# jianwang-mpi/SceneEgo

Measured on NVIDIA B200. Metric: frames/s VoxelNetDepth volumetric stage, higher is better.
Workload: dtype bf16

## Files before the change

sceneego_b200/build.py:

```python
import concurrent.futures
import hashlib
import os
import subprocess
import sys

HERE = os.path.dirname(os.path.abspath(__file__))
CSRC = os.path.join(HERE, "csrc")
LIB = os.path.join(HERE, "libsceneego_b200.so")
LIB_F16 = os.path.join(HERE, "libsceneego_b200_f16.so")
HASH_FILE = LIB + ".srchash"
OBJ_DIR = os.path.join(HERE, "build")
SOURCES = ["geometry.cu", "softargmax.cu", "v2v.cu", "stem.cu", "stem_march.cu", "tail.cu", "march.cu", "eval.cu", "handoff.cu", "feature_conv.cu"]
NVCC_FLAGS = ["-gencode", "arch=compute_100a,code=sm_100a", "-O3", "-lineinfo", "-std=c++17",
              "-Xcompiler", "-fPIC", "-Xptxas", "-v"]


def _sources():
    return [s for s in SOURCES if os.path.exists(os.path.join(CSRC, s))]


def source_hash() -> str:
    h = hashlib.sha256()
    deps = sorted(os.path.join(CSRC, f) for f in os.listdir(CSRC) if f.endswith((".cu", ".cuh", ".h")))
    deps.append(os.path.join(HERE, "..", "include", "sceneego_b200.h"))
    for d in deps:
        h.update(os.path.basename(d).encode())
        h.update(open(d, "rb").read())
    h.update(" ".join(NVCC_FLAGS + _sources()).encode())
    return h.hexdigest()


def recorded_hash() -> str:
    try:
        return open(HASH_FILE).read().strip()
    except OSError:
        return ""


def _stale() -> bool:
    return not (os.path.exists(LIB) and os.path.exists(LIB_F16)) or recorded_hash() != source_hash()


VARIANTS = [("bf16", LIB, []), ("f16", LIB_F16, ["-DSCENEEGO_ACT_F16"])]


# ... 40 lines not shown
```

sceneego_b200/csrc/common.cuh:

```cuda
#pragma once
#include <cuda_runtime.h>
#include <cuda_bf16.h>
#include <cuda_fp16.h>
#include <stdint.h>
#include <stdio.h>
#include "../../include/sceneego_b200.h"

namespace sceneego {

#ifdef SCENEEGO_ACT_F16
constexpr int kActDtype = 1;
constexpr uint32_t kIdescAB = 0u;
#define SE_MMA_SYNC_AB ".f16.f16"
__device__ __forceinline__ uint32_t act_pack2(float lo, float hi) {
  uint32_t r;
  asm("cvt.rn.satfinite.f16x2.f32 %0, %1, %2;" : "=r"(r) : "f"(hi), "f"(lo));
  return r;
}
__device__ __forceinline__ uint32_t act_pack2_relu(float lo, float hi) {
  uint32_t r;
  asm("cvt.rn.relu.satfinite.f16x2.f32 %0, %1, %2;" : "=r"(r) : "f"(hi), "f"(lo));
  return r;
}
__device__ __forceinline__ float2 act_unpack2(uint32_t u) { return __half22float2(*reinterpret_cast<const __half2*>(&u)); }
// ... 62 lines not shown
}

__device__ __forceinline__ float voxel_coord(float lo, float step, int i) {
  return __fadd_rn(lo, __fmul_rn(step, (float)i));
}

__host__ __device__ inline int64_t vol_cell(const sceneego_vol_layout_t& L, int b, int x, int y, int z, int g, int C8) {
  if (L.s2d) {
    const int par = ((x & 1) << 2) | ((y & 1) << 1) | (z & 1);
    return (int64_t)(par * C8 + g) * L.plane_stride + vol_pos(L, b, x >> 1, y >> 1, z >> 1);
  }
  return (int64_t)g * L.plane_stride + vol_pos(L, b, x, y, z);
}
__host__ __device__ inline int64_t vol_scene_elem(const sceneego_vol_layout_t& L, int b, int x, int y, int z, int C8) {
  if (L.s2d) {
    const int par = ((x & 1) << 2) | ((y & 1) << 1) | (z & 1);
    return ((int64_t)(8 * C8) * L.plane_stride + vol_pos(L, b, x >> 1, y >> 1, z >> 1)) * 8 + par;
  }
  return ((int64_t)C8 * L.plane_stride + vol_pos(L, b, x, y, z)) * 8;
}

constexpr int kNumSMs = 148;

int launch_stem_s2d(const sceneego_v2v_op_t& op, void* const* d_buffers, const void* d_blob, int batch, int op_index,
                    bool simt, cudaStream_t st);
int launch_feature_conv1x1_simt(const float* d_feat, const float* d_weight, const float* d_bias, float* d_out, int batch,
                                int cin, int cout, int h, int w, cudaStream_t st);
int launch_stem_march(const sceneego_v2v_op_t& op, void* const* d_buffers, const void* d_blob, int batch, int op_index,
                      bool simt, cudaStream_t st);
int launch_tail_mlp(const sceneego_v2v_op_t& op, void* const* d_buffers, const void* d_blob, int batch, int op_index,
                    bool simt, cudaStream_t st);
int launch_conv_march(const sceneego_v2v_op_t& op, void* const* d_buffers, const void* d_blob, int batch, int op_index,
                      cudaStream_t st);

}
```

sceneego_b200/csrc/v2v.cu:

```cuda
#include "tc_common.cuh"
#include <stdarg.h>
#include <stdlib.h>
#include <string.h>
#include <math.h>
#include <mutex>

namespace sceneego {


struct ConvParams {
  const __nv_bfloat16* src;
  __nv_bfloat16* dst;
  const __nv_bfloat16* res;
  float* dst_f32;
  const __nv_bfloat16* w;
  const float* bias;
  sceneego_vol_layout_t ls, ld;
  int batch;
  int k, r, cin_planes, ksteps, N, cout_real, flags;
  int xs, n0, n_dx, n_xg, items_per_plane;
  FastDiv fd_frame, fd_px, fd_py;
  int deconv, par0;
  int taps_dx;
  int mma_n;
  int tiles, L, WL;
  int n_items;
  int win_stages, w_slots, wchunk_taps, wchunks_per_dx;
  int wrows;
  uint32_t win_bytes, wchunk_bytes, tap_bytes;
  uint32_t off_win, off_w, off_bias, off_bar;
  uint32_t tmem_cols, half_cols;
  int cg;
  uint32_t w_half_bytes;
  const __nv_bfloat16* src2;
  int n_dx2;
  uint32_t w_main_bytes;
  int march;
  int n0_shift;
};

constexpr int CONV_EPI_WARPS = 8;
__host__ __device__ constexpr int conv_mma_warps(int tiles) { return tiles >= 4 ? 4 : tiles; }
__host__ __device__ constexpr int conv_threads(int tiles) { return 32 * (1 + conv_mma_warps(tiles) + CONV_EPI_WARPS); }
constexpr int CONV_MAX_THREADS = 32 * (1 + 4 + CONV_EPI_WARPS);
constexpr int MAX_STAGES = 4, MAX_WSLOTS = 8;

struct RowInfo {
  bool write;
  bool valid;
  int b, n;
  int x, y, z;
  int64_t dpos;
};

__device__ __forceinline__ RowInfo decode_row(const ConvParams& p, int64_t q64) {
  RowInfo ri;
  ri.write = false; ri.valid = false; ri.b = 0; ri.n = 0; ri.dpos = 0; ri.x = ri.y = ri.z = 0;
  const int S = p.ls.side;
  const uint32_t q = (uint32_t)q64;
  const uint32_t b = fdiv(q, p.fd_frame);
  const int rem = (int)(q - b * (uint32_t)p.ls.frame_pitch) - p.ls.guard;
  if ((int)b >= p.batch || rem < 0) return ri;
  const int x = (int)fdiv((uint32_t)rem, p.fd_px);
  const int r2 = rem - x * p.ls.pitch_x;
  const int y = (int)fdiv((uint32_t)r2, p.fd_py);
  const int z = r2 - y * p.ls.pitch_y;
  if (x >= S) return ri;
  if (y >= S + p.ld.pad || z >= S + p.ld.pad) return ri;
  ri.write = true;
  ri.valid = (y < S) && (z < S);
  ri.b = (int)b;
  ri.x = x; ri.y = y; ri.z = z;
  ri.n = (x * S + y) * S + z;
  const int m = p.deconv ? 2 : 1;
  ri.dpos = (int64_t)b * p.ld.frame_pitch + p.ld.guard + (int64_t)(m * x) * p.ld.pitch_x + (int64_t)(m * y) * p.ld.pitch_y + m * z;
  return ri;
}

__device__ __forceinline__ RowInfo decode_row_plane(const ConvParams& p, int b, int x, int cell) {
  RowInfo ri;
  ri.write = false; ri.valid = false; ri.b = b; ri.n = 0; ri.dpos = 0; ri.x = x; ri.y = ri.z = 0;
  const int S = p.ls.side;
  if (cell >= p.ls.pitch_x) return ri;
  const int y = (int)fdiv((uint32_t)cell, p.fd_py);
  const int z = cell - y * p.ls.pitch_y;
  if (y >= S + p.ld.pad || z >= S + p.ld.pad) return ri;
  ri.write = true;
  ri.valid = (y < S) && (z < S);
  ri.y = y; ri.z = z;
  ri.n = (x * S + y) * S + z;
  ri.dpos = (int64_t)b * p.ld.frame_pitch + p.ld.guard + (int64_t)x * p.ld.pitch_x + (int64_t)y * p.ld.pitch_y + z;
  return ri;
}

__device__ __forceinline__ void store_row16_pre(const ConvParams& p, const RowInfo& ri, int c0, float (&v)[16],
                                                const float* s_bias, const uint4& r0, const uint4& r1) {
  if (!ri.write) return;
  const int S = p.ls.side;
  if (p.flags & SCENEEGO_F_OUT_F32) {
    if (!ri.valid) return;
    const size_t N3 = (size_t)S * S * S;
#pragma unroll
    for (int j = 0; j < 16; ++j) {
      const int c = c0 + j;
      if (c < p.cout_real) {
        float o = v[j] + s_bias[c];
        if (p.flags & SCENEEGO_F_RELU) o = fmaxf(o, 0.f);
        p.dst_f32[((size_t)ri.b * p.cout_real + c) * N3 + ri.n] = o;
// ... 172 lines not shown
          }
          for (int e = 0; e < p.n_dx2; ++e) {
            mbar_wait(BAR(B_FULL_WIN + ws), wph);
            mbar_arrive_remote(mapa_shared(BAR(B_FULL_WIN + ws), 0));
            if (++ws == p.win_stages) { ws = 0; wph ^= 1; }
            mbar_wait(BAR(B_FULL_W + sl), sph);
            mbar_arrive_remote(mapa_shared(BAR(B_FULL_W + sl), 0));
            if (++sl == p.w_slots) { sl = 0; sph ^= 1; }
          }
        }
      }
    } else {
    const uint32_t tmem_u = __shfl_sync(0xffffffffu, tmem_base, 0);
    const bool leader = elect_one();
    auto WAIT = [&](uint32_t bar, uint32_t parity) {
      if constexpr (CG == 2) mbar_wait_warp_cluster(bar, parity); else mbar_wait_warp(bar, parity);
    };
    auto MMA = [&](uint32_t d, uint64_t a, uint64_t b, uint32_t id, uint32_t ac) {
      if constexpr (CG == 2) tc_mma_bf16_pair(d, a, b, id, ac); else tc_mma_bf16(d, a, b, id, ac);
    };
    auto COMMIT = [&](uint32_t bar) {
      if constexpr (CG == 2) tc_commit_pair(bar); else tc_commit(bar);
    };
    const uint32_t idesc = (1u << 4) | kIdescAB | ((uint32_t)(p.mma_n >> 3) << 17) | ((CG == 2 ? 16u : 8u) << 24);
    const uint64_t desc_hi = (uint64_t)(8u | (1u << 14)) << 32;
    const uint32_t a_lo_flags = ((p.win_bytes >> 4) & 0x3FFFu) << 16;
    const uint32_t n_mine = (uint32_t)p.mma_n / CG;
    const uint32_t b_lo_flags = ((n_mine * 16u >> 4) & 0x3FFFu) << 16;
    const uint32_t a_ks_step = (2u * p.win_bytes) >> 4;
    const uint32_t b_ks_step = (2u * n_mine * 16u) >> 4;
    const uint32_t b_tap_step = p.tap_bytes >> 4;
    const uint32_t n_cols = (uint32_t)p.N;
    const int pitch_y = p.ls.pitch_y, ksz = p.k, wtaps = p.wchunk_taps;
    const uint32_t is_deconv = (uint32_t)p.deconv, par_cols = (uint32_t)p.n0;
    const uint32_t my_tile = (uint32_t)(warp - 1);
    const uint32_t a_mine = my_tile * 128u;
    int ws = 0, wph = 0, sl = 0, sph = 0;
    for (int it = 0; it < my_items; ++it) {
      const int buf = it & 1;
      WAIT(BAR(B_TMEM_EMPTY + buf), ((it >> 1) & 1) ^ 1);
      tc_fence_after();
      const uint32_t d_mine = tmem_u + (uint32_t)buf * p.half_cols + my_tile * n_cols;
      uint32_t acc = 0;
      for (int dx = 0; dx < p.n_dx; ++dx) {
        WAIT(BAR(B_FULL_WIN + ws), wph);
        const uint32_t win_lo = (((sbase + p.off_win + (uint32_t)(ws * 2 * KSTEPS) * p.win_bytes) >> 4) & 0x3FFFu) |
                                a_lo_flags;
        int dy = 0, dz = 0;
        uint32_t dcol = 0;
        for (int wc = 0; wc < p.wchunks_per_dx; ++wc) {
          WAIT(BAR(B_FULL_W + sl), sph);
          tc_fence_after();
          uint32_t b_lo = (((sbase + p.off_w + (uint32_t)sl * p.wchunk_bytes) >> 4) & 0x3FFFu) | b_lo_flags;
          if constexpr (WROWS == 0) {
            for (int tp = 0; tp < wtaps; ++tp) {
              const uint32_t a_lo = win_lo + (uint32_t)(dy * pitch_y + dz);
              if (leader) {
#pragma unroll
                for (int tt = 0; tt < TILES / NW; ++tt) {
#pragma unroll
                  for (int ks = 0; ks < KSTEPS; ++ks)
                    MMA(d_mine + (uint32_t)(tt * NW) * n_cols + dcol,
                                desc_hi | (a_lo + a_mine + (uint32_t)(tt * NW) * 128u + (uint32_t)ks * a_ks_step),
                                desc_hi | (b_lo + (uint32_t)ks * b_ks_step), idesc, ks == 0 ? acc : 1u);
                }
              }
              b_lo += b_tap_step;
              if (is_deconv) { dcol += par_cols; }
              else { acc = 1; if (++dz == ksz) { dz = 0; ++dy; } }
            }
          } else {
            if (leader) {
#pragma unroll
              for (int r = 0; r < WROWS; ++r) {
                const uint32_t a_row = win_lo + a_mine + (uint32_t)((dy + r) * pitch_y);
#pragma unroll
                for (int j = 0; j < 3; ++j) {
#pragma unroll
                  for (int tt = 0; tt < TILES / NW; ++tt) {
#pragma unroll
                    for (int ks = 0; ks < KSTEPS; ++ks)
                      MMA(d_mine + (uint32_t)(tt * NW) * n_cols,
                                  desc_hi | (a_row + (uint32_t)j + (uint32_t)(tt * NW) * 128u + (uint32_t)ks * a_ks_step),
                                  desc_hi | (b_lo + (uint32_t)(r * 3 + j) * b_tap_step + (uint32_t)ks * b_ks_step), idesc,
                                  (ks == 0 && r == 0 && j == 0) ? acc : 1u);
                  }
                }
              }
            }
            acc = 1;
            dy += WROWS;
          }
          if (leader) COMMIT(BAR(B_EMPTY_W + sl));
          if (++sl == p.w_slots) { sl = 0; sph ^= 1; }
        }
        if (leader) COMMIT(BAR(B_EMPTY_WIN + ws));
        if (++ws == p.win_stages) { ws = 0; wph ^= 1; }
      }
      if constexpr (KSTEPS % 2 == 0) {
        for (int e = 0; e < p.n_dx2; ++e) {
          WAIT(BAR(B_FULL_WIN + ws), wph);
          WAIT(BAR(B_FULL_W + sl), sph);
          tc_fence_after();
          const uint32_t a_c = ((((sbase + p.off_win + (uint32_t)(ws * 2 * KSTEPS) * p.win_bytes) >> 4) & 0x3FFFu) | a_lo_flags) +
                               a_mine + (uint32_t)(p.r * (pitch_y + 1));
          const uint32_t b_c = (((sbase + p.off_w + (uint32_t)sl * p.wchunk_bytes) >> 4) & 0x3FFFu) | b_lo_flags;
          if (leader) {
#pragma unroll
            for (int tt = 0; tt < TILES / NW; ++tt) {
#pragma unroll
              for (int ks = 0; ks < KSTEPS / 2; ++ks)
                MMA(d_mine + (uint32_t)(tt * NW) * n_cols, desc_hi | (a_c + (uint32_t)(tt * NW) * 128u + (uint32_t)ks * a_ks_step),
                    desc_hi | (b_c + (uint32_t)ks * b_ks_step), idesc, 1u);
            }
          }
          if (leader) COMMIT(BAR(B_EMPTY_W + sl));
          if (++sl == p.w_slots) { sl = 0; sph ^= 1; }
          if (leader) COMMIT(BAR(B_EMPTY_WIN + ws));
          if (++ws == p.win_stages) { ws = 0; wph ^= 1; }
        }
      }
      if (leader) COMMIT(BAR(B_TMEM_FULL + buf));
    }
    __syncwarp();
    }
  } else {
    const int quarter = warp & 3;
    const int half = (warp - FIRST_EPI) >> 2;
    const int nch = p.N >> 4;
    const int S = p.ls.side;
    const int t_first = TILES >= 2 ? half : 0, t_step = TILES >= 2 ? 2 : 1;
    const int c_first = TILES >= 2 ? 0 : half, c_step = TILES >= 2 ? 1 : 2;
    auto shifted = [&](const RowInfo& ri, int x0, int c, int& ch0) -> RowInfo {
      if (XS == 1 && p.deconv) {
        const int blk = p.n0_shift >= 0 ? ((c << 4) >> p.n0_shift) : (c << 4) / p.n0;
        const int par = p.par0 + blk;
        ch0 = (c << 4) - blk * p.n0;
        RowInfo r = ri;
        r.write = ri.valid;
        r.dpos = ri.dpos + ((par >> 2) * p.ld.pitch_x + ((par >> 1) & 1) * p.ld.pitch_y + (par & 1));
        return r;
      }
      if (XS == 1) { ch0 = c << 4; return ri; }
      const int sft = p.n0_shift >= 0 ? ((c << 4) >> p.n0_shift) : (c << 4) / p.n0;
      ch0 = (c << 4) - sft * p.n0;
      RowInfo r = ri;
      const bool in = (x0 + sft) < S;
      r.write = ri.write && in;
      r.valid = ri.valid && in;
      r.dpos = ri.dpos + (int64_t)sft * p.ld.pitch_x;
      r.n = ri.n + sft * S * S;
      return r;
    };
    for (int it = 0; it < my_items; ++it) {
      const int buf = it & 1;
      int ib, ix0, icell0;
      const int64_t q0 = item_origin(item_of(it), ib, ix0, icell0);
      auto row_info = [&](int t) -> RowInfo {
        const int r = t * 128 + quarter * 32 + lane;
        return XS == 1 ? decode_row(p, q0 + r) : decode_row_plane(p, ib, ix0, icell0 + r);
      };
      RowInfo ri = row_info(t_first);
      if constexpr (TILES == 1) {
        constexpr int D = 4;
        uint4 q0r[D], q1r[D];
#pragma unroll
        for (int d = 0; d < D; ++d) {
          q0r[d] = make_uint4(0, 0, 0, 0); q1r[d] = q0r[d];
          const int c = c_first + d * c_step;
          if (c < nch) { int chn; const RowInfo rp = shifted(ri, ix0, c, chn); load_res16(p, rp, chn, q0r[d], q1r[d]); }
        }
        mbar_wait(BAR(B_TMEM_FULL + buf), (it >> 1) & 1);
        tc_fence_after();
        const uint32_t taddr = tmem_base + ((uint32_t)(quarter * 32) << 16) + (uint32_t)buf * p.half_cols;
        int cpf = c_first + D * c_step;
// ... 165 lines not shown
  const int So = ld.side;
  const int n = blockIdx.x * blockDim.x + threadIdx.x;
  const int g = blockIdx.y, b = blockIdx.z;
  if (n >= So * So * So || g >= planes) return;
  const int z = n % So, y = (n / So) % So, x = n / (So * So);
  float m[8];
#pragma unroll
  for (int j = 0; j < 8; ++j) m[j] = -INFINITY;
#pragma unroll
  for (int t = 0; t < 8; ++t) {
    const int64_t q = vol_pos(ls, b, 2 * x + (t >> 2), 2 * y + ((t >> 1) & 1), 2 * z + (t & 1));
    float a[8];
    unpack8(*reinterpret_cast<const uint4*>(src + ((int64_t)g * ls.plane_stride + q) * 8), a);
#pragma unroll
    for (int j = 0; j < 8; ++j) m[j] = fmaxf(m[j], a[j]);
  }
  *reinterpret_cast<uint4*>(dst + ((int64_t)g * ld.plane_stride + vol_pos(ld, b, x, y, z)) * 8) = pack8(m);
}

__global__ void __launch_bounds__(128) deconv2_kernel(const __grid_constant__ ConvParams p) {
  const int So = p.ld.side;
  const int n = blockIdx.x * blockDim.x + threadIdx.x;
  const int go = blockIdx.y, b = blockIdx.z;
  if (n >= So * So * So) return;
  const int z = n % So, y = (n / So) % So, x = n / (So * So);
  const int tap = ((x & 1) * 2 + (y & 1)) * 2 + (z & 1);
  const int64_t qs = vol_pos(p.ls, b, x >> 1, y >> 1, z >> 1);
  float acc[8];
#pragma unroll
  for (int j = 0; j < 8; ++j) acc[j] = 0.f;
  for (int g = 0; g < p.cin_planes; ++g) {
    float a[8];
    unpack8(*reinterpret_cast<const uint4*>(p.src + ((int64_t)g * p.ls.plane_stride + qs) * 8), a);
    int npar = 256 / p.N;
    if (npar > 8) npar = 8;
    const uint4* wrow = reinterpret_cast<const uint4*>(p.w) +
                        ((size_t)(tap / npar) * p.cin_planes + g) * ((size_t)npar * p.N) + (size_t)(tap % npar) * p.N + go * 8;
#pragma unroll
    for (int j = 0; j < 8; ++j) {
      float wv[8];
      unpack8(__ldg(wrow + j), wv);
#pragma unroll
      for (int i = 0; i < 8; ++i) acc[j] = fmaf(a[i], wv[i], acc[j]);
    }
  }
  const int64_t cell = (int64_t)go * p.ld.plane_stride + vol_pos(p.ld, b, x, y, z);
  float rr[8];
  if (p.flags & SCENEEGO_F_ADD_AFTER) unpack8(*reinterpret_cast<const uint4*>(p.res + cell * 8), rr);
#pragma unroll
  for (int j = 0; j < 8; ++j) {
    float t = acc[j] + p.bias[go * 8 + j];
    if (p.flags & SCENEEGO_F_RELU) t = fmaxf(t, 0.f);
    if (p.flags & SCENEEGO_F_ADD_AFTER) t += rr[j];
    acc[j] = t;
  }
  *reinterpret_cast<uint4*>(p.dst + cell * 8) = pack8(acc);
}

static thread_local char g_err[512] = "";
int ensure_max_dynamic_smem(const void* kernel, int bytes) {
  struct Entry { int dev; const void* fn; int bytes; };
  static Entry seen[512];
  static int n_seen = 0;
  static std::mutex mu;
  int dev = 0;
  cudaError_t e = cudaGetDevice(&dev);
  if (e != cudaSuccess) { set_error("cudaGetDevice: %s", cudaGetErrorString(e)); return SCENEEGO_E_CUDA; }
  std::lock_guard<std::mutex> lock(mu);
  for (int i = 0; i < n_seen; ++i)
    if (seen[i].dev == dev && seen[i].fn == kernel && seen[i].bytes >= bytes) return SCENEEGO_OK;
  e = cudaFuncSetAttribute(kernel, cudaFuncAttributeMaxDynamicSharedMemorySize, bytes);
  if (e != cudaSuccess) { set_error("cudaFuncSetAttribute(MaxDynamicSharedMemorySize): %s", cudaGetErrorString(e)); return SCENEEGO_E_CUDA; }
  if (n_seen < 512) seen[n_seen++] = Entry{dev, kernel, bytes};
  return SCENEEGO_OK;
}

void set_error(const char* fmt, ...) {
  va_list ap;
  va_start(ap, fmt);
  vsnprintf(g_err, sizeof(g_err), fmt, ap);
  va_end(ap);
}
static thread_local int g_launches = 0;

static bool try_plan(ConvParams& p, int tiles, int want_stages) {
  const int taps_dx = p.taps_dx;
  const int L = tiles * 128;
  const int WL = L + 2 * p.r * (p.ls.pitch_y + 1);
  const uint32_t win_bytes = (uint32_t)WL * 16u;
  const uint32_t stage = win_bytes * p.cin_planes;
  const uint32_t fixed = 1024;
  if ((uint64_t)stage * want_stages + fixed > kMaxSmem) return false;
  const uint32_t used = stage * want_stages + fixed;
  const uint32_t room = kMaxSmem - used;
  int wct = taps_dx, wrows = 0;
  if (p.k == 3 && !p.deconv && 3u * 9u * p.tap_bytes <= room) { wct = 9; wrows = 3; }
  else if (p.k == 3 && !p.deconv && 2u * 3u * p.tap_bytes <= room) { wct = 3; wrows = 1; }
  else {
    while (wct > 1 && (uint32_t)wct * p.tap_bytes > 24576u) {
      int nx = wct - 1;
      while (nx > 1 && taps_dx % nx) --nx;
      wct = nx;
    }
  }
  { const char* e = getenv("SCENEEGO_WCHUNK"); if (e && atoi(e) > 0 && taps_dx % atoi(e) == 0) { wct = atoi(e); wrows = (p.k == 3 && !p.deconv && wct % 3 == 0) ? wct / 3 : 0; if (wrows == 2) wrows = 0; } }
  const uint32_t wchunk = (uint32_t)wct * p.tap_bytes;
  if (2ull * wchunk > room) return false;
  int slots = (int)(room / wchunk);
  if (slots > MAX_WSLOTS) slots = MAX_WSLOTS;
  if (slots > 4 && wchunk > 8192) slots = 4;
  { const char* e = getenv("SCENEEGO_WSLOTS"); if (e && atoi(e) >= 2 && atoi(e) <= MAX_WSLOTS && (uint64_t)used + (uint64_t)atoi(e) * wchunk <= kMaxSmem) slots = atoi(e); }
  p.wrows = wrows;
  p.tiles = tiles; p.L = L; p.WL = WL;
  p.win_bytes = win_bytes; p.win_stages = want_stages;
  p.wchunk_taps = wct; p.wchunks_per_dx = taps_dx / wct; p.wchunk_bytes = wchunk; p.w_slots = slots;
  p.off_win = 0;
  p.off_w = stage * want_stages;
  p.off_bias = p.off_w + wchunk * slots;
  p.off_bar = p.off_bias + 512;
  p.half_cols = (uint32_t)(tiles * p.N);
  uint32_t cols = 32;
  while (cols < 2 * p.half_cols) cols <<= 1;
  p.tmem_cols = cols;
  return true;
}

static int plan_conv(ConvParams& p, int64_t n_pos) {
  p.tap_bytes = (uint32_t)p.cin_planes * (p.mma_n / p.cg) * 16u;
  int max_tiles = 256 / p.N;
  if (max_tiles > 8) max_tiles = 8;
  if (p.xs == 1 && p.cg == 1) {
    auto items_of = [&](int t) { return (n_pos + (int64_t)t * 128 - 1) / ((int64_t)t * 128); };
    if (items_of(max_tiles) < 4 * kNumSMs) {
      int best = max_tiles;
      int64_t best_cost = ((items_of(max_tiles) + kNumSMs - 1) / kNumSMs) * max_tiles;
      for (int t = max_tiles >> 1; t >= 1; t >>= 1) {
        const int64_t cost = ((items_of(t) + kNumSMs - 1) / kNumSMs) * t;
        if (cost < best_cost) { best_cost = cost; best = t; }
// ... 26 lines not shown
extern "C" int sceneego_v2v_last_launch_count(void) { return g_launches; }

extern "C" int sceneego_v2v_pack_conv(const float* h_weight, const float* h_bias, const float* h_gamma,
                                      const float* h_beta, const float* h_mean, const float* h_var, double eps,
                                      int cout, int cin, int ksize, int transposed, int cout_pad, int cin_pad,
                                      int xstack, int n_split, uint16_t* h_w_out, float* h_b_out) {
  SE_REQUIRE(h_weight && h_w_out && h_b_out, "pack_conv: null argument");
  SE_REQUIRE(cout_pad >= cout && cin_pad >= cin && cout_pad % 8 == 0 && cin_pad % 8 == 0, "pack_conv: bad padding");
  SE_REQUIRE(xstack >= 1 && (xstack == 1 || !transposed), "pack_conv: bad xstack");
  SE_REQUIRE(n_split == 1 || (n_split == 2 && !transposed && (xstack * cout_pad) % 32 == 0), "pack_conv: bad n_split");
  const int taps = ksize * ksize * ksize;
  const int kk = ksize * ksize;
  const int n_stk = xstack * cout_pad;
  const int n_dx = ksize + xstack - 1;
  memset(h_w_out, 0, (size_t)n_dx * kk * cin_pad * n_stk * sizeof(uint16_t));
  for (int co = 0; co < cout_pad; ++co) {
    double scale = 1.0, shift = 0.0;
    if (co < cout) {
      if (h_gamma) {
        scale = (double)h_gamma[co] / sqrt((double)h_var[co] + eps);
        shift = (double)h_beta[co] - (double)h_mean[co] * scale;
      }
      h_b_out[co] = (float)((h_bias ? (double)h_bias[co] : 0.0) * scale + shift);
    } else {
      h_b_out[co] = 0.f;
    }
    if (co >= cout) continue;
    for (int ci = 0; ci < cin; ++ci)
      for (int t = 0; t < taps; ++t) {
        const size_t src = transposed ? (((size_t)ci * cout + co) * taps + t) : (((size_t)co * cin + ci) * taps + t);
        const uint16_t wv = f2bf((float)((double)h_weight[src] * scale));
        const int dx = t / kk, rest = t % kk;
        if (transposed) {
          int npar = 256 / cout_pad;
          if (npar > 8) npar = 8;
          const size_t grp = (size_t)t / npar, nrow = (size_t)(t % npar) * cout_pad + co;
          h_w_out[((grp * (cin_pad / 8) + ci / 8) * ((size_t)npar * cout_pad) + nrow) * 8 + (ci & 7)] = wv;
          continue;
        }
        for (int sft = 0; sft < xstack; ++sft) {
          const size_t tp = (size_t)(dx + sft) * kk + rest;
          const size_t col = (size_t)sft * cout_pad + co;
          const size_t nh = (size_t)n_stk / n_split, hf = col / nh;
          const size_t half_elems = (size_t)n_dx * kk * cin_pad * nh;
          const size_t dst = hf * half_elems + ((tp * (cin_pad / 8) + ci / 8) * nh + (col - hf * nh)) * 8 + (ci & 7);
          h_w_out[dst] = wv;
        }
      }
  }
  return SCENEEGO_OK;
}

static int launch_conv_tc(ConvParams& p, int batch, int op_index, cudaStream_t st) {
  p.n0_shift = -1;
  for (int k = 3; k < 10; ++k) if ((1 << k) == p.n0) p.n0_shift = k;
  const int64_t n_pos = (int64_t)batch * p.ls.frame_pitch;
  SE_REQUIRE(n_pos + 4096 < (1ll << 31) && (n_pos + 4096) * (int64_t)p.ls.frame_pitch < (1ll << 48),
             "v2v_run: op %d: batch * frame_pitch too large for one launch (use a smaller chunk)", op_index);
  p.fd_frame = make_fastdiv((uint32_t)p.ls.frame_pitch);
  p.fd_px = make_fastdiv((uint32_t)p.ls.pitch_x);
  p.fd_py = make_fastdiv((uint32_t)p.ls.pitch_y);
  const int smem = plan_conv(p, n_pos);
  SE_REQUIRE(smem > 0, "v2v_run: op %d does not fit shared memory", op_index);
  if (p.xs == 1) {
    p.n_items = (int)((n_pos + p.L - 1) / p.L);
  } else {
    p.items_per_plane = (p.ls.pitch_x + p.L - 1) / p.L;
    p.n_xg = (p.ls.side + p.xs - 1) / p.xs;
// ... 45 lines not shown
    ConvParams p;
    memset(&p, 0, sizeof(p));
    p.src = (const __nv_bfloat16*)d_buffers[op.src];
    p.dst = (__nv_bfloat16*)d_buffers[op.dst];
    p.dst_f32 = (float*)d_buffers[op.dst];
    p.res = op.res >= 0 ? (const __nv_bfloat16*)d_buffers[op.res] : nullptr;
    p.ls = op.lay_src; p.ld = op.lay_dst; p.batch = batch; p.flags = op.flags;
    SE_REQUIRE(p.src && p.dst, "v2v_run: op %d has a null buffer", i);
    SE_REQUIRE(!(op.flags & (SCENEEGO_F_RESIDUAL | SCENEEGO_F_ADD_AFTER)) || p.res, "v2v_run: op %d needs a residual", i);
    if (op.type == SCENEEGO_OP_MAXPOOL2) {
      SE_REQUIRE(op.lay_dst.side * 2 == op.lay_src.side && op.cin % 8 == 0, "v2v_run: op %d bad pool shape", i);
      const int So = op.lay_dst.side;
      dim3 grid((So * So * So + 255) / 256, op.cin / 8, batch);
      maxpool2_kernel<<<grid, 256, 0, st>>>(p.src, p.dst, p.ls, p.ld, op.cin / 8);
      SE_CUDA_LAUNCH_CHECK("maxpool2");
      ++g_launches;
      continue;
    }
    if (op.type == SCENEEGO_OP_STEM7_S2D || op.type == SCENEEGO_OP_TAIL_MLP || op.type == SCENEEGO_OP_STEM7_MARCH) {
      const bool simt = op.impl == 1 || force_simt;
      const int rc = op.type == SCENEEGO_OP_STEM7_S2D ? launch_stem_s2d(op, d_buffers, d_blob, batch, i, simt, st)
                     : op.type == SCENEEGO_OP_STEM7_MARCH ? launch_stem_march(op, d_buffers, d_blob, batch, i, simt, st)
                                                          : launch_tail_mlp(op, d_buffers, d_blob, batch, i, simt, st);
      if (rc != SCENEEGO_OK) return rc;
      ++g_launches;
      continue;
    }
    p.w = (const __nv_bfloat16*)((const char*)d_blob + op.w_offset);
    p.bias = (const float*)((const char*)d_blob + op.b_offset);
    p.cin_planes = op.cin / 8; p.ksteps = op.cin / 16; p.N = op.cout; p.cout_real = op.cout_real;
    p.xs = 1; p.n0 = op.cout; p.n_dx = op.ksize; p.n_xg = 0; p.items_per_plane = 0; p.cg = 1;
    if (op.type == SCENEEGO_OP_DECONV2) {
      SE_REQUIRE(op.lay_dst.side == 2 * op.lay_src.side && op.cin % 8 == 0 && op.cout % 8 == 0, "v2v_run: op %d bad deconv shape", i);
      if (op.impl == 1 || force_simt || op.cin % 16 || op.cout % 16 || op.cout > 256) {
        const int So = op.lay_dst.side;
        dim3 grid((So * So * So + 127) / 128, op.cout / 8, batch);
        deconv2_kernel<<<grid, 128, 0, st>>>(p);
        SE_CUDA_LAUNCH_CHECK("deconv2");
        ++g_launches;
        continue;
      }
      int npar = 256 / op.cout;
      if (npar > 8) npar = 8;
      const __nv_bfloat16* w_all = p.w;
      for (int par0 = 0; par0 < 8; par0 += npar) {
        ConvParams q = p;
        q.k = 1; q.r = 0; q.xs = 1; q.n0 = op.cout; q.mma_n = npar * op.cout; q.N = npar * op.cout; q.n_dx = 1;
        q.deconv = 1; q.par0 = par0; q.taps_dx = 1;
        q.w = w_all + (size_t)par0 * q.cin_planes * op.cout * 8;
        const int rc = launch_conv_tc(q, batch, i, st);
        if (rc != SCENEEGO_OK) return rc;
      }
      continue;
    }
    if (op.type == SCENEEGO_OP_CONV3_MARCH) {
      if (op.impl == 1 || force_simt) {
        SE_REQUIRE(op.ksize == 3 && op.cin % 16 == 0 && op.cout % 16 == 0, "v2v_run: op %d bad marching conv", i);
        p.k = 3; p.r = 1; p.xs = 1; p.n0 = op.cout; p.N = op.cout; p.cg = 1; p.march = 1;
        p.fd_frame = make_fastdiv((uint32_t)p.ls.frame_pitch);
        p.fd_px = make_fastdiv((uint32_t)p.ls.pitch_x);
        p.fd_py = make_fastdiv((uint32_t)p.ls.pitch_y);
        p.src2 = nullptr; p.n_dx2 = 0;
        if (op.src2 >= 0 && op.cin2 > 0) { p.src2 = (const __nv_bfloat16*)d_buffers[op.src2]; p.n_dx2 = 1; }
        p.w_main_bytes = 27u * (uint32_t)p.cin_planes * (uint32_t)op.cout * 16u;
        p.w_half_bytes = 0;
        const int64_t n_pos = (int64_t)batch * p.ls.frame_pitch;
        dim3 grid((unsigned)((n_pos + 127) / 128), op.cout / 16);
        conv_simt_kernel<<<grid, 128, 0, st>>>(p, n_pos);
        SE_CUDA_LAUNCH_CHECK("conv_simt (march layout)");
      } else {
        const int rc = launch_conv_march(op, d_buffers, d_blob, batch, i, st);
        if (rc != SCENEEGO_OK) return rc;
      }
      ++g_launches;
      continue;
    }
    SE_REQUIRE(op.type == SCENEEGO_OP_CONV, "v2v_run: op %d unknown type", i);
    SE_REQUIRE(op.ksize == 1 || op.ksize == 3 || op.ksize == 7, "v2v_run: op %d unsupported kernel size", i);
    SE_REQUIRE(op.cin % 16 == 0 && op.cout % 16 == 0 && op.cout >= 16 && op.cout <= 128, "v2v_run: op %d channels must be multiples of 16", i);
    SE_REQUIRE(op.lay_src.side == op.lay_dst.side && op.lay_src.pad >= op.ksize / 2 && op.lay_dst.pad <= op.lay_src.pad,
               "v2v_run: op %d layouts incompatible with the stencil", i);
    p.k = op.ksize; p.r = op.ksize / 2;
    const int64_t n_pos = (int64_t)batch * p.ls.frame_pitch;
    p.fd_frame = make_fastdiv((uint32_t)p.ls.frame_pitch);
    p.fd_px = make_fastdiv((uint32_t)p.ls.pitch_x);
    p.fd_py = make_fastdiv((uint32_t)p.ls.pitch_y);
    p.cg = op.cta_pair == 2 ? 2 : 1;
    p.src2 = nullptr; p.n_dx2 = 0;
    if (op.src2 >= 0 && op.cin2 > 0) {
      SE_REQUIRE(op.cin2 * 2 == op.cin && (op.cin / 16) % 2 == 0 && op.ksize == 3 && d_buffers[op.src2],
                 "v2v_run: op %d: a fused shortcut needs a 3^3 conv and a second source with half its channels", i);
      p.src2 = (const __nv_bfloat16*)d_buffers[op.src2];
      p.n_dx2 = op.xstack > 1 ? op.xstack : 1;
    }
    if (op.impl == 1 || force_simt) {
      const int xs_ = op.xstack > 1 ? op.xstack : 1;
      p.n0 = op.cout; p.N = xs_ * op.cout;
      const uint32_t tapb = (uint32_t)p.cin_planes * (p.N / p.cg) * 16u;
      p.w_main_bytes = (uint32_t)((op.ksize + xs_ - 1) * op.ksize * op.ksize) * tapb;
      p.w_half_bytes = p.w_main_bytes + (uint32_t)p.n_dx2 * (tapb / 2);
      dim3 grid((unsigned)((n_pos + 127) / 128), op.cout / 16);
      conv_simt_kernel<<<grid, 128, 0, st>>>(p, n_pos);
      SE_CUDA_LAUNCH_CHECK("conv_simt");
      ++g_launches;
      continue;
    }
    const int xs = op.xstack > 1 ? op.xstack : 1;
    SE_REQUIRE(xs * op.cout <= 256, "v2v_run: op %d: xstack * cout exceeds 256 columns", i);
    SE_REQUIRE(p.cg == 1 || (xs * op.cout) % 32 == 0, "v2v_run: op %d: a CTA pair splits N in halves of whole 16-column groups", i);
    p.xs = xs; p.n0 = op.cout; p.N = xs * op.cout; p.mma_n = p.N; p.n_dx = op.ksize + xs - 1;
    p.deconv = 0; p.par0 = 0; p.taps_dx = op.ksize * op.ksize;
    const int rc = launch_conv_tc(p, batch, i, st);
    if (rc != SCENEEGO_OK) return rc;
  }
  if (ev) cudaEventRecord(ev[n_ops], st);
  return SCENEEGO_OK;
}

extern "C" int sceneego_v2v_run(const sceneego_v2v_op_t* ops, int n_ops, void* const* d_buffers, const void* d_blob,
                                int batch, void* stream) {
  return v2v_run_impl(ops, n_ops, d_buffers, d_blob, batch, stream, nullptr);
}

extern "C" int sceneego_v2v_run_profile(const sceneego_v2v_op_t* ops, int n_ops, void* const* d_buffers,
                                        const void* d_blob, int batch, void* stream, float* h_ms) {
  SE_REQUIRE(h_ms && n_ops > 0 && n_ops < 4096, "v2v_run_profile: bad argument");
  cudaEvent_t* ev = (cudaEvent_t*)malloc(sizeof(cudaEvent_t) * (n_ops + 1));
  for (int i = 0; i <= n_ops; ++i) cudaEventCreate(&ev[i]);
  int rc = v2v_run_impl(ops, n_ops, d_buffers, d_blob, batch, stream, ev);
  if (rc == SCENEEGO_OK) {
    cudaError_t e = cudaEventSynchronize(ev[n_ops]);
    if (e != cudaSuccess) { set_error("v2v_run_profile: %s", cudaGetErrorString(e)); rc = SCENEEGO_E_CUDA; }
    for (int i = 0; i < n_ops && rc == SCENEEGO_OK; ++i) cudaEventElapsedTime(&h_ms[i], ev[i], ev[i + 1]);
  }
  for (int i = 0; i <= n_ops; ++i) cudaEventDestroy(ev[i]);
  free(ev);
  return rc;
}
```

Measured before the change: 2992.

## Add dedicated warp-specialized tcgen05 transposed-conv kernel with smem-staged bulk stores

Replaces the per-parity-group launches of the generic tensor-core conv for 2x transposed convolutions with one persistent warp-specialized kernel. A producer warp streams input windows, weights and optional residual tiles through mbarrier pipelines, and an MMA warp accumulates into double-buffered TMEM. Sixteen epilogue warps scatter results into a shared-memory output image that a storer warp writes back with bulk async copies. The aim is to cut multiple launches, reread source data less often and coalesce the strided parity writes. The cost is considerable new synchronization complexity and a deconv path removed from the generic kernel.

```diff
diff --git a/sceneego_b200/build.py b/sceneego_b200/build.py
--- a/sceneego_b200/build.py
+++ b/sceneego_b200/build.py
@@ -10,7 +10,7 @@
 LIB_F16 = os.path.join(HERE, "libsceneego_b200_f16.so")
 HASH_FILE = LIB + ".srchash"
 OBJ_DIR = os.path.join(HERE, "build")
-SOURCES = ["geometry.cu", "softargmax.cu", "v2v.cu", "stem.cu", "stem_march.cu", "tail.cu", "march.cu", "eval.cu", "handoff.cu", "feature_conv.cu"]
+SOURCES = ["geometry.cu", "softargmax.cu", "v2v.cu", "stem.cu", "stem_march.cu", "tail.cu", "march.cu", "eval.cu", "handoff.cu", "feature_conv.cu", "deconv.cu"]
 NVCC_FLAGS = ["-gencode", "arch=compute_100a,code=sm_100a", "-O3", "-lineinfo", "-std=c++17",
               "-Xcompiler", "-fPIC", "-Xptxas", "-v"]
 
diff --git a/sceneego_b200/csrc/common.cuh b/sceneego_b200/csrc/common.cuh
--- a/sceneego_b200/csrc/common.cuh
+++ b/sceneego_b200/csrc/common.cuh
@@ -118,5 +118,8 @@
                     bool simt, cudaStream_t st);
 int launch_conv_march(const sceneego_v2v_op_t& op, void* const* d_buffers, const void* d_blob, int batch, int op_index,
                       cudaStream_t st);
+__host__ __device__ inline int deconv_npar(int cout) { return 256 / cout < 8 ? 256 / cout : 8; }
+int launch_deconv_tc(const sceneego_v2v_op_t& op, void* const* d_buffers, const void* d_blob, int batch, int op_index,
+                     cudaStream_t st);
 
 }
diff --git a/sceneego_b200/csrc/deconv.cu b/sceneego_b200/csrc/deconv.cu
--- /dev/null
+++ b/sceneego_b200/csrc/deconv.cu
@@ -0,0 +1,298 @@
+#include "tc_common.cuh"
+
+namespace sceneego {
+
+constexpr int DC_EPI_WARPS = 16;
+constexpr int DC_THREADS = 32 * (2 + DC_EPI_WARPS);
+constexpr int DC_MAX_IMG = 3;
+
+struct DeconvParams {
+  const __nv_bfloat16* src;
+  const __nv_bfloat16* res;
+  __nv_bfloat16* dst;
+  const uint8_t* w;
+  const float* bias;
+  sceneego_vol_layout_t ls, ld;
+  int flags, ksteps, cout, npar, n_groups, nl, items_per_plane, n_items, n_img;
+  uint32_t group_bytes, win_plane_bytes, img_bytes, tmem_cols;
+  uint32_t off_win, off_img, off_w, off_bias, off_bar;
+  int win_stages;
+};
+
+__device__ __forceinline__ void bulk_s2g(void* dst, uint32_t src, uint32_t bytes) {
+  asm volatile("cp.async.bulk.global.shared::cta.bulk_group [%0], [%1], %2;" ::"l"(dst), "r"(src), "r"(bytes) : "memory");
+}
+
+__global__ void __launch_bounds__(DC_THREADS, 1) deconv_tc_kernel(const __grid_constant__ DeconvParams p) {
+  extern __shared__ __align__(128) uint8_t smem[];
+  const int warp = __shfl_sync(0xffffffffu, (int)(threadIdx.x >> 5), 0);
+  const int lane = threadIdx.x & 31;
+  const uint32_t sbase = smem_u32(smem);
+  float* s_bias = reinterpret_cast<float*>(smem + p.off_bias);
+  const uint32_t bar0 = sbase + p.off_bar;
+  auto BAR = [&](int i) { return bar0 + 8u * (uint32_t)i; };
+  constexpr int B_W_FULL = 0, B_W_EMPTY = 2, B_WIN_FULL = 4, B_WIN_EMPTY = 6, B_TM_FULL = 8, B_TM_EMPTY = 10,
+                B_IMG_FULL = 12, B_IMG_EMPTY = B_IMG_FULL + DC_MAX_IMG, B_COUNT = B_IMG_EMPTY + DC_MAX_IMG;
+  uint32_t* s_tmem_ptr = reinterpret_cast<uint32_t*>(smem + p.off_bar + 8 * B_COUNT);
+
+  const int S = p.ls.side, py = p.ls.pitch_y;
+  const int N = p.npar * p.cout;
+  const int cpl = p.cout >> 3;
+  const int gpi = p.npar == 2 ? 2 : 1;
+  const int n_ranges = (p.npar == 8 ? 2 : 1) * cpl;
+  const int pyd = p.ld.pitch_y;
+  const uint32_t range_bytes = (uint32_t)(2 * p.nl * pyd) * 16u;
+  const bool resident = p.n_groups <= 2;
+
+  for (int i = threadIdx.x; i < p.cout; i += DC_THREADS) s_bias[i] = p.bias[i];
+  if (threadIdx.x == 0) {
+    for (int i = 0; i < 2; ++i) {
+      mbar_init(BAR(B_W_FULL + i), 1); mbar_init(BAR(B_W_EMPTY + i), 1);
+      mbar_init(BAR(B_WIN_FULL + i), 1); mbar_init(BAR(B_WIN_EMPTY + i), 1);
+      mbar_init(BAR(B_TM_FULL + i), 1); mbar_init(BAR(B_TM_EMPTY + i), DC_EPI_WARPS);
+    }
+    for (int i = 0; i < DC_MAX_IMG; ++i) { mbar_init(BAR(B_IMG_FULL + i), 1); mbar_init(BAR(B_IMG_EMPTY + i), 1); }
+    asm volatile("fence.mbarrier_init.release.cluster;" ::: "memory");
+  }
+  if (warp == 1) {
+    asm volatile("tcgen05.alloc.cta_group::1.sync.aligned.shared::cta.b32 [%0], %1;" ::"r"(smem_u32(s_tmem_ptr)), "r"(p.tmem_cols)
+                 : "memory");
+    asm volatile("tcgen05.relinquish_alloc_permit.cta_group::1.sync.aligned;" ::: "memory");
+  }
+  tc_fence_before();
+  __syncthreads();
+  tc_fence_after();
+  const uint32_t tmem_base = *s_tmem_ptr;
+
+  const int my_items = (p.n_items - (int)blockIdx.x + (int)gridDim.x - 1) / (int)gridDim.x;
+  auto item_of = [&](int it, int& b, int& x, int& y0, int& nli) {
+    const int item = (int)blockIdx.x + it * (int)gridDim.x;
+    const int t = item / p.items_per_plane;
+    y0 = (item - t * p.items_per_plane) * p.nl;
+    x = t % S; b = t / S;
+    nli = min(p.nl, S - y0);
+  };
+  auto range_cell = [&](int b, int x, int y0, int gi, int r) -> int64_t {
+    const int i = ((gi * p.npar) >> 2) + r / cpl;
+    return (int64_t)(r % cpl) * p.ld.plane_stride + vol_pos(p.ld, b, 2 * x + i, 2 * y0, 0);
+  };
+  auto range_copy_bytes = [&](int nli) { return (uint32_t)((2 * nli - 1) * pyd + 2 * S) * 16u; };
+
+  if (warp == 0) {
+    auto expect = [&](uint32_t bar, uint32_t bytes) {
+      if (lane == 0) mbar_expect_tx(bar, bytes);
+      __syncwarp();
+    };
+    if (resident) {
+      expect(BAR(B_W_FULL), p.group_bytes * (uint32_t)p.n_groups);
+      if (lane < p.n_groups) bulk_g2s(sbase + p.off_w + (uint32_t)lane * p.group_bytes, p.w + (size_t)lane * p.group_bytes,
+                                      p.group_bytes, BAR(B_W_FULL));
+    }
+    const bool skip = (p.flags & SCENEEGO_F_ADD_AFTER) != 0;
+    uint32_t k = 0, m = 0;
+    for (int it = 0; it < my_items; ++it) {
+      int b, x, y0, nli;
+      item_of(it, b, x, y0, nli);
+      const int ws = it % p.win_stages;
+      mbar_wait(BAR(B_WIN_EMPTY + ws), ((it / p.win_stages) & 1) ^ 1);
+      expect(BAR(B_WIN_FULL + ws), (uint32_t)(nli * py) * 16u * (uint32_t)(2 * p.ksteps));
+      const int64_t q0 = vol_pos(p.ls, b, x, y0, 0);
+      for (int g = lane; g < 2 * p.ksteps; g += 32)
+        bulk_g2s(sbase + p.off_win + (uint32_t)(ws * 2 * p.ksteps + g) * p.win_plane_bytes,
+                 p.src + ((int64_t)g * p.ls.plane_stride + q0) * 8, (uint32_t)(nli * py) * 16u, BAR(B_WIN_FULL + ws));
+      const uint32_t cb = range_copy_bytes(nli);
+      for (int gi = 0; gi < p.n_groups; ++gi, ++k) {
+        if (!resident) {
+          const int s = (int)(k & 1u);
+          mbar_wait(BAR(B_W_EMPTY + s), ((k >> 1) & 1u) ^ 1u);
+          expect(BAR(B_W_FULL + s), p.group_bytes);
+          if (lane == 0)
+            bulk_g2s(sbase + p.off_w + (uint32_t)s * p.group_bytes, p.w + (size_t)gi * p.group_bytes, p.group_bytes, BAR(B_W_FULL + s));
+        }
+        if (gi % gpi) continue;
+        const int is = (int)(m % (uint32_t)p.n_img);
+        mbar_wait(BAR(B_IMG_EMPTY + is), ((m / (uint32_t)p.n_img) & 1u) ^ 1u);
+        if (skip) {
+          const uint32_t img = sbase + p.off_img + (uint32_t)is * p.img_bytes;
+          expect(BAR(B_IMG_FULL + is), (uint32_t)n_ranges * cb);
+          for (int r = lane; r < n_ranges; r += 32)
+            bulk_g2s(img + (uint32_t)r * range_bytes, p.res + range_cell(b, x, y0, gi, r) * 8, cb, BAR(B_IMG_FULL + is));
+        } else if (lane == 0) {
+          mbar_arrive(BAR(B_IMG_FULL + is));
+        }
+        ++m;
+      }
+    }
+  } else if (warp == 1) {
+    const uint32_t tmem_u = __shfl_sync(0xffffffffu, tmem_base, 0);
+    const bool leader = elect_one();
+    const uint32_t idesc = (1u << 4) | kIdescAB | ((uint32_t)(N >> 3) << 17) | (8u << 24);
+    const uint64_t desc_hi = (uint64_t)(8u | (1u << 14)) << 32;
+    const uint32_t a_flags = ((p.win_plane_bytes >> 4) & 0x3FFFu) << 16;
+    const uint32_t b_flags = (((uint32_t)N * 16u >> 4) & 0x3FFFu) << 16;
+    const uint32_t a_ks = (2u * p.win_plane_bytes) >> 4, b_ks = (2u * (uint32_t)N * 16u) >> 4;
+    if (resident) mbar_wait_warp(BAR(B_W_FULL), 0);
+    uint32_t k = 0;
+    for (int it = 0; it < my_items; ++it) {
+      const int ws = it % p.win_stages;
+      mbar_wait_warp(BAR(B_WIN_FULL + ws), (uint32_t)(it / p.win_stages) & 1u);
+      const uint32_t a_lo = (((sbase + p.off_win + (uint32_t)(ws * 2 * p.ksteps) * p.win_plane_bytes) >> 4) & 0x3FFFu) | a_flags;
+      for (int gi = 0; gi < p.n_groups; ++gi, ++k) {
+        const uint32_t h = k & 1u;
+        const uint32_t slot = resident ? (uint32_t)gi : h;
+        mbar_wait_warp(BAR(B_TM_EMPTY + (int)h), ((k >> 1) & 1u) ^ 1u);
+        if (!resident) mbar_wait_warp(BAR(B_W_FULL + (int)slot), (k >> 1) & 1u);
+        tc_fence_after();
+        const uint32_t b_lo = (((sbase + p.off_w + slot * p.group_bytes) >> 4) & 0x3FFFu) | b_flags;
+        if (leader) {
+          for (int ks = 0; ks < p.ksteps; ++ks)
+            tc_mma_bf16(tmem_u + h * (uint32_t)N, desc_hi | (a_lo + (uint32_t)ks * a_ks), desc_hi | (b_lo + (uint32_t)ks * b_ks),
+                        idesc, ks == 0 ? 0u : 1u);
+          if (!resident) tc_commit(BAR(B_W_EMPTY + (int)slot));
+          if (gi == p.n_groups - 1) tc_commit(BAR(B_WIN_EMPTY + ws));
+          tc_commit(BAR(B_TM_FULL + (int)h));
+        }
+        __syncwarp();
+      }
+    }
+  } else {
+    const int quarter = warp & 3;
+    const int sub = (warp - 2) >> 2;
+    const int row = quarter * 32 + lane;
+    const int t_row = row / py, z_row = row - t_row * py;
+    const bool relu = (p.flags & SCENEEGO_F_RELU) != 0;
+    const bool add_after = (p.flags & SCENEEGO_F_ADD_AFTER) != 0;
+    const bool storer = warp == 2;
+    const int nch = N >> 4;
+    const uint32_t lane_base = tmem_base + ((uint32_t)(quarter * 32) << 16);
+    auto finish16 = [&](uint8_t* img, int gi, int c0, const uint32_t (&raw)[16], bool pad) {
+      const int par_l = c0 / p.cout, ch0 = c0 - par_l * p.cout;
+      const int par = gi * p.npar + par_l;
+      if (pad && (par & 1)) return;
+      const int ii = (par >> 2) - ((gi * p.npar) >> 2);
+      const int cell = (2 * t_row + ((par >> 1) & 1)) * pyd + 2 * z_row + (par & 1);
+#pragma unroll
+      for (int g = 0; g < 2; ++g) {
+        const int r = ii * cpl + (ch0 >> 3) + g;
+        uint4* ptr = reinterpret_cast<uint4*>(img + (size_t)r * range_bytes + (size_t)cell * 16);
+        if (pad) { *ptr = make_uint4(0, 0, 0, 0); continue; }
+        float rr[8];
+        if (add_after) unpack8(*ptr, rr);
+        const float4 b0 = *reinterpret_cast<const float4*>(s_bias + ch0 + 8 * g);
+        const float4 b1 = *reinterpret_cast<const float4*>(s_bias + ch0 + 8 * g + 4);
+        const float bs[8] = {b0.x, b0.y, b0.z, b0.w, b1.x, b1.y, b1.z, b1.w};
+        float o[8];
+#pragma unroll
+        for (int j = 0; j < 8; ++j) {
+          float t = __uint_as_float(raw[8 * g + j]) + bs[j];
+          if (relu) t = fmaxf(t, 0.f);
+          if (add_after) t += rr[j];
+          o[j] = t;
+        }
+        *ptr = pack8(o);
+      }
+    };
+    uint32_t k = 0, m = 0;
+    for (int it = 0; it < my_items; ++it) {
+      int b, x, y0, nli;
+      item_of(it, b, x, y0, nli);
+      const bool valid = t_row < nli && z_row <= S, pad = z_row == S;
+      for (int gi = 0; gi < p.n_groups; ++gi, ++k) {
+        const uint32_t h = k & 1u;
+        const int is = (int)(m % (uint32_t)p.n_img);
+        uint8_t* img = smem + p.off_img + (size_t)is * p.img_bytes;
+        mbar_wait(BAR(B_TM_FULL + (int)h), (k >> 1) & 1u);
+        if (gi % gpi == 0) mbar_wait(BAR(B_IMG_FULL + is), (m / (uint32_t)p.n_img) & 1u);
+        tc_fence_after();
+        const uint32_t taddr = lane_base + h * (uint32_t)N;
+#pragma unroll 1
+        for (int c = sub; c < nch; c += 8) {
+          uint32_t ra[16], rb[16];
+          const bool two = c + 4 < nch;
+          tc_ld16(taddr + (uint32_t)(c << 4), ra);
+          if (two) tc_ld16(taddr + (uint32_t)((c + 4) << 4), rb);
+          tc_wait_ld();
+          if (valid) {
+            finish16(img, gi, c << 4, ra, pad);
+            if (two) finish16(img, gi, (c + 4) << 4, rb, pad);
+          }
+        }
+        tc_fence_before();
+        __syncwarp();
+        if (lane == 0) mbar_arrive(BAR(B_TM_EMPTY + (int)h));
+        if (gi % gpi != gpi - 1) continue;
+        asm volatile("fence.proxy.async.shared::cta;" ::: "memory");
+        asm volatile("bar.sync 1, %0;" ::"n"(32 * DC_EPI_WARPS) : "memory");
+        if (storer) {
+          const uint32_t simg = sbase + p.off_img + (uint32_t)is * p.img_bytes;
+          for (int r = lane; r < n_ranges; r += 32)
+            bulk_s2g(p.dst + range_cell(b, x, y0, gi, r) * 8, simg + (uint32_t)r * range_bytes, range_copy_bytes(nli));
+          asm volatile("cp.async.bulk.commit_group;" ::: "memory");
+          asm volatile("cp.async.bulk.wait_group.read 1;" ::: "memory");
+          __syncwarp();
+          if (lane == 0 && m > 0) mbar_arrive(BAR(B_IMG_EMPTY + (int)((m - 1) % (uint32_t)p.n_img)));
+        }
+        ++m;
+      }
+    }
+    if (storer) asm volatile("cp.async.bulk.wait_group 0;" ::: "memory");
+  }
+  tc_fence_before();
+  __syncthreads();
+  if (warp == 1)
+    asm volatile("tcgen05.dealloc.cta_group::1.sync.aligned.b32 %0, %1;" ::"r"(tmem_base), "r"(p.tmem_cols) : "memory");
+}
+
+int launch_deconv_tc(const sceneego_v2v_op_t& op, void* const* d_buffers, const void* d_blob, int batch, int op_index,
+                     cudaStream_t st) {
+  DeconvParams p;
+  memset(&p, 0, sizeof(p));
+  p.src = (const __nv_bfloat16*)d_buffers[op.src];
+  p.dst = (__nv_bfloat16*)d_buffers[op.dst];
+  p.res = op.res >= 0 ? (const __nv_bfloat16*)d_buffers[op.res] : nullptr;
+  p.w = (const uint8_t*)d_blob + op.w_offset;
+  p.bias = (const float*)((const char*)d_blob + op.b_offset);
+  p.ls = op.lay_src; p.ld = op.lay_dst; p.flags = op.flags;
+  const int S = p.ls.side, py = p.ls.pitch_y;
+  SE_REQUIRE(op.cin % 16 == 0 && op.cout % 16 == 0 && deconv_npar(op.cout) % 2 == 0 && p.ls.s2d == 0 && p.ld.s2d == 0,
+             "v2v_run: op %d: no deconv_tc_kernel for cin=%d cout=%d", op_index, op.cin, op.cout);
+  SE_REQUIRE(p.ls.pad >= 1 && p.ld.pad == 1, "v2v_run: op %d: deconv_tc_kernel needs pad 1 layouts", op_index);
+  p.ksteps = op.cin / 16;
+  p.cout = op.cout;
+  p.npar = deconv_npar(op.cout);
+  p.n_groups = 8 / p.npar;
+  const int cin_planes = op.cin / 8, N = p.npar * p.cout;
+  p.group_bytes = (uint32_t)cin_planes * (uint32_t)N * 16u;
+  p.tmem_cols = 32;
+  while (p.tmem_cols < 2u * (uint32_t)N) p.tmem_cols <<= 1;
+  const uint32_t w_bytes = (uint32_t)(p.n_groups <= 2 ? p.n_groups : 2) * p.group_bytes;
+  const uint32_t line_img = (uint32_t)((p.npar == 8 ? 2 : 1) * (p.cout / 8)) * (uint32_t)(2 * p.ld.pitch_y) * 16u;
+  size_t smem = 0;
+  for (int nl = (128 / py < S ? 128 / py : S); nl >= 1 && !smem; --nl)
+    for (int n_img = DC_MAX_IMG; n_img >= 2 && !smem; --n_img)
+      for (int stages = 2; stages >= 1 && !smem; --stages) {
+        const uint64_t plane = (uint64_t)(nl * py + 7) / 8 * 128;
+        const uint64_t off_img = (uint64_t)stages * cin_planes * plane, img = (uint64_t)nl * line_img;
+        const uint64_t off_w = (off_img + n_img * img + 127) / 128 * 128;
+        const uint64_t end = off_w + w_bytes + 512 + 512;
+        if (end > kMaxSmem) continue;
+        p.nl = nl; p.n_img = n_img; p.win_stages = stages; p.win_plane_bytes = (uint32_t)plane; p.img_bytes = (uint32_t)img;
+        p.off_win = 0; p.off_img = (uint32_t)off_img; p.off_w = (uint32_t)off_w;
+        p.off_bias = p.off_w + w_bytes;
+        p.off_bar = p.off_bias + 512u;
+        smem = (size_t)end;
+      }
+  SE_REQUIRE(smem > 0, "v2v_run: op %d: transposed conv (cin %d, side %d) does not fit shared memory", op_index, op.cin, S);
+  if (smem < kMaxSmem / 2 + 1024) smem = kMaxSmem / 2 + 1024;
+  p.items_per_plane = (S + p.nl - 1) / p.nl;
+  const int64_t n_items = (int64_t)batch * S * p.items_per_plane;
+  SE_REQUIRE(n_items < (1ll << 31), "v2v_run: op %d: batch too large for one launch", op_index);
+  p.n_items = (int)n_items;
+  const int grid = p.n_items < kNumSMs ? p.n_items : kNumSMs;
+  if (int rc = ensure_max_dynamic_smem((const void*)deconv_tc_kernel, (int)kMaxSmem)) return rc;
+  deconv_tc_kernel<<<grid, DC_THREADS, smem, st>>>(p);
+  SE_CUDA_LAUNCH_CHECK("deconv_tc");
+  return SCENEEGO_OK;
+}
+
+}
diff --git a/sceneego_b200/csrc/v2v.cu b/sceneego_b200/csrc/v2v.cu
--- a/sceneego_b200/csrc/v2v.cu
+++ b/sceneego_b200/csrc/v2v.cu
@@ -20,7 +20,6 @@
   int k, r, cin_planes, ksteps, N, cout_real, flags;
   int xs, n0, n_dx, n_xg, items_per_plane;
   FastDiv fd_frame, fd_px, fd_py;
-  int deconv, par0;
   int taps_dx;
   int mma_n;
   int tiles, L, WL;
@@ -72,8 +71,7 @@
   ri.b = (int)b;
   ri.x = x; ri.y = y; ri.z = z;
   ri.n = (x * S + y) * S + z;
-  const int m = p.deconv ? 2 : 1;
-  ri.dpos = (int64_t)b * p.ld.frame_pitch + p.ld.guard + (int64_t)(m * x) * p.ld.pitch_x + (int64_t)(m * y) * p.ld.pitch_y + m * z;
+  ri.dpos = (int64_t)b * p.ld.frame_pitch + p.ld.guard + (int64_t)x * p.ld.pitch_x + (int64_t)y * p.ld.pitch_y + z;
   return ri;
 }
 
@@ -312,7 +310,6 @@
     const uint32_t b_tap_step = p.tap_bytes >> 4;
     const uint32_t n_cols = (uint32_t)p.N;
     const int pitch_y = p.ls.pitch_y, ksz = p.k, wtaps = p.wchunk_taps;
-    const uint32_t is_deconv = (uint32_t)p.deconv, par_cols = (uint32_t)p.n0;
     const uint32_t my_tile = (uint32_t)(warp - 1);
     const uint32_t a_mine = my_tile * 128u;
     int ws = 0, wph = 0, sl = 0, sph = 0;
@@ -327,7 +324,6 @@
         const uint32_t win_lo = (((sbase + p.off_win + (uint32_t)(ws * 2 * KSTEPS) * p.win_bytes) >> 4) & 0x3FFFu) |
                                 a_lo_flags;
         int dy = 0, dz = 0;
-        uint32_t dcol = 0;
         for (int wc = 0; wc < p.wchunks_per_dx; ++wc) {
           WAIT(BAR(B_FULL_W + sl), sph);
           tc_fence_after();
@@ -340,14 +336,14 @@
                 for (int tt = 0; tt < TILES / NW; ++tt) {
 #pragma unroll
                   for (int ks = 0; ks < KSTEPS; ++ks)
-                    MMA(d_mine + (uint32_t)(tt * NW) * n_cols + dcol,
+                    MMA(d_mine + (uint32_t)(tt * NW) * n_cols,
                                 desc_hi | (a_lo + a_mine + (uint32_t)(tt * NW) * 128u + (uint32_t)ks * a_ks_step),
                                 desc_hi | (b_lo + (uint32_t)ks * b_ks_step), idesc, ks == 0 ? acc : 1u);
                 }
               }
               b_lo += b_tap_step;
-              if (is_deconv) { dcol += par_cols; }
-              else { acc = 1; if (++dz == ksz) { dz = 0; ++dy; } }
+              acc = 1;
+              if (++dz == ksz) { dz = 0; ++dy; }
             }
           } else {
             if (leader) {
@@ -412,15 +408,6 @@
     const int t_first = TILES >= 2 ? half : 0, t_step = TILES >= 2 ? 2 : 1;
     const int c_first = TILES >= 2 ? 0 : half, c_step = TILES >= 2 ? 1 : 2;
     auto shifted = [&](const RowInfo& ri, int x0, int c, int& ch0) -> RowInfo {
-      if (XS == 1 && p.deconv) {
-        const int blk = p.n0_shift >= 0 ? ((c << 4) >> p.n0_shift) : (c << 4) / p.n0;
-        const int par = p.par0 + blk;
-        ch0 = (c << 4) - blk * p.n0;
-        RowInfo r = ri;
-        r.write = ri.valid;
-        r.dpos = ri.dpos + ((par >> 2) * p.ld.pitch_x + ((par >> 1) & 1) * p.ld.pitch_y + (par & 1));
-        return r;
-      }
       if (XS == 1) { ch0 = c << 4; return ri; }
       const int sft = p.n0_shift >= 0 ? ((c << 4) >> p.n0_shift) : (c << 4) / p.n0;
       ch0 = (c << 4) - sft * p.n0;
@@ -652,8 +639,7 @@
   for (int g = 0; g < p.cin_planes; ++g) {
     float a[8];
     unpack8(*reinterpret_cast<const uint4*>(p.src + ((int64_t)g * p.ls.plane_stride + qs) * 8), a);
-    int npar = 256 / p.N;
-    if (npar > 8) npar = 8;
+    const int npar = deconv_npar(p.N);
     const uint4* wrow = reinterpret_cast<const uint4*>(p.w) +
                         ((size_t)(tap / npar) * p.cin_planes + g) * ((size_t)npar * p.N) + (size_t)(tap % npar) * p.N + go * 8;
 #pragma unroll
@@ -714,8 +700,8 @@
   const uint32_t used = stage * want_stages + fixed;
   const uint32_t room = kMaxSmem - used;
   int wct = taps_dx, wrows = 0;
-  if (p.k == 3 && !p.deconv && 3u * 9u * p.tap_bytes <= room) { wct = 9; wrows = 3; }
-  else if (p.k == 3 && !p.deconv && 2u * 3u * p.tap_bytes <= room) { wct = 3; wrows = 1; }
+  if (p.k == 3 && 3u * 9u * p.tap_bytes <= room) { wct = 9; wrows = 3; }
+  else if (p.k == 3 && 2u * 3u * p.tap_bytes <= room) { wct = 3; wrows = 1; }
   else {
     while (wct > 1 && (uint32_t)wct * p.tap_bytes > 24576u) {
       int nx = wct - 1;
@@ -723,7 +709,7 @@
       wct = nx;
     }
   }
-  { const char* e = getenv("SCENEEGO_WCHUNK"); if (e && atoi(e) > 0 && taps_dx % atoi(e) == 0) { wct = atoi(e); wrows = (p.k == 3 && !p.deconv && wct % 3 == 0) ? wct / 3 : 0; if (wrows == 2) wrows = 0; } }
+  { const char* e = getenv("SCENEEGO_WCHUNK"); if (e && atoi(e) > 0 && taps_dx % atoi(e) == 0) { wct = atoi(e); wrows = (p.k == 3 && wct % 3 == 0) ? wct / 3 : 0; if (wrows == 2) wrows = 0; } }
   const uint32_t wchunk = (uint32_t)wct * p.tap_bytes;
   if (2ull * wchunk > room) return false;
   int slots = (int)(room / wchunk);
@@ -816,8 +802,7 @@
         const uint16_t wv = f2bf((float)((double)h_weight[src] * scale));
         const int dx = t / kk, rest = t % kk;
         if (transposed) {
-          int npar = 256 / cout_pad;
-          if (npar > 8) npar = 8;
+          const int npar = deconv_npar(cout_pad);
           const size_t grp = (size_t)t / npar, nrow = (size_t)(t % npar) * cout_pad + co;
           h_w_out[((grp * (cin_pad / 8) + ci / 8) * ((size_t)npar * cout_pad) + nrow) * 8 + (ci & 7)] = wv;
           continue;
@@ -929,7 +914,8 @@
     p.xs = 1; p.n0 = op.cout; p.n_dx = op.ksize; p.n_xg = 0; p.items_per_plane = 0; p.cg = 1;
     if (op.type == SCENEEGO_OP_DECONV2) {
       SE_REQUIRE(op.lay_dst.side == 2 * op.lay_src.side && op.cin % 8 == 0 && op.cout % 8 == 0, "v2v_run: op %d bad deconv shape", i);
-      if (op.impl == 1 || force_simt || op.cin % 16 || op.cout % 16 || op.cout > 256) {
+      SE_REQUIRE(!(op.flags & ~(SCENEEGO_F_RELU | SCENEEGO_F_ADD_AFTER)), "v2v_run: op %d: a transposed conv takes only RELU and ADD_AFTER", i);
+      if (op.impl == 1 || force_simt || op.cin % 16 || op.cout % 16 || op.cout > 256 || deconv_npar(op.cout) % 2) {
         const int So = op.lay_dst.side;
         dim3 grid((So * So * So + 127) / 128, op.cout / 8, batch);
         deconv2_kernel<<<grid, 128, 0, st>>>(p);
@@ -937,17 +923,9 @@
         ++g_launches;
         continue;
       }
-      int npar = 256 / op.cout;
-      if (npar > 8) npar = 8;
-      const __nv_bfloat16* w_all = p.w;
-      for (int par0 = 0; par0 < 8; par0 += npar) {
-        ConvParams q = p;
-        q.k = 1; q.r = 0; q.xs = 1; q.n0 = op.cout; q.mma_n = npar * op.cout; q.N = npar * op.cout; q.n_dx = 1;
-        q.deconv = 1; q.par0 = par0; q.taps_dx = 1;
-        q.w = w_all + (size_t)par0 * q.cin_planes * op.cout * 8;
-        const int rc = launch_conv_tc(q, batch, i, st);
-        if (rc != SCENEEGO_OK) return rc;
-      }
+      const int rc = launch_deconv_tc(op, d_buffers, d_blob, batch, i, st);
+      if (rc != SCENEEGO_OK) return rc;
+      ++g_launches;
       continue;
     }
     if (op.type == SCENEEGO_OP_CONV3_MARCH) {
@@ -1006,7 +984,7 @@
     SE_REQUIRE(xs * op.cout <= 256, "v2v_run: op %d: xstack * cout exceeds 256 columns", i);
     SE_REQUIRE(p.cg == 1 || (xs * op.cout) % 32 == 0, "v2v_run: op %d: a CTA pair splits N in halves of whole 16-column groups", i);
     p.xs = xs; p.n0 = op.cout; p.N = xs * op.cout; p.mma_n = p.N; p.n_dx = op.ksize + xs - 1;
-    p.deconv = 0; p.par0 = 0; p.taps_dx = op.ksize * op.ksize;
+    p.taps_dx = op.ksize * op.ksize;
     const int rc = launch_conv_tc(p, batch, i, st);
     if (rc != SCENEEGO_OK) return rc;
   }
```

After: 3050 (median of 6 runs). 1.02x the previous value.
